# bassamlab/SigmaRL

Measured on AMD Instinct MI355X. Metric: env-steps/sec (agents x envs x steps), CPM scenario, 16 agents (open loop, 32 steps per launch), higher is better.
Workload: dtype f32

## Files before the change

sigmarl_amd/csrc/sigmaenv.hip:

```cpp
#include <hip/hip_runtime.h>

#include <algorithm>
#include <atomic>
#include <cmath>
#include <cstdio>
#include <cstdlib>
#include <cstring>
#include <string>
#include <type_traits>
#include <vector>

#include "sigmaenv_device.h"

using namespace sigmadev;

#ifdef SIGMAENV_PROFILE
#define PROF_TS2(g, tid, k) do { if ((g).dbg_ts2 && (tid) == 0) (g).dbg_ts2[(size_t)blockIdx.x * 16 + (k)] = __builtin_readcyclecounter(); } while (0)
#else
#define PROF_TS2(g, tid, k) do { } while (0)
#endif

#include "../../include/sigmaenv_ref_weights.h"
static_assert(NS >= 1 && NS <= SIGMAENV_MAX_SHORT_TERM, "SIGMAENV_N_SHORT_TERM out of range");
__device__ __constant__ uint32_t W_REF_BITS[NS] = SIGMAENV_W_REF_BITS;
// ... 1032 lines not shown
  for (int k = threadIdx.x; k < t.slots * NS * 2; k += blockDim.x) s.shrt[k] = g.short_term[t.a0 * NS * 2 + k];
  for (int k = threadIdx.x; k < t.slots; k += blockDim.x) s.dref[k] = g.dist_ref[t.a0 + k];
  for (int k = threadIdx.x; k < t.slots * 5; k += blockDim.x) { s.dleft[k] = g.dist_left[t.a0 * 5 + k]; s.dright[k] = g.dist_right[t.a0 * 5 + k]; }
  for (int k = threadIdx.x; k < t.slots * N; k += blockDim.x) s.dist[(k / N) * DIST_STRIDE(N) + (k % N)] = g.dist_agents[t.a0 * N + k];
  for (int k = threadIdx.x; k < t.slots; k += blockDim.x) {
    float psi = g.state[(t.a0 + k) * 8 + 2];
    s.cs[k * 2] = cr_cos(psi);
    s.cs[k * 2 + 1] = cr_sin(psi);
    s.path[k] = g.path[(t.a0 + k) * 4];
    s.cp[k * 3 + 0] = g.closest[(t.a0 + k) * 3 + 0]; s.cp[k * 3 + 1] = g.closest[(t.a0 + k) * 3 + 1]; s.cp[k * 3 + 2] = g.closest[(t.a0 + k) * 3 + 2];
    s.fresh[k] = g.fresh ? g.fresh[t.a0 + k] : 0;
  }
  __syncthreads();
}

__global__ void __launch_bounds__(256) sigmaenv_observe_kernel(sigmaenv_config_t c, DevBufs g, int G) {
  sigma_poison_lds();
  extern __shared__ __attribute__((aligned(16))) char smem_raw[];
  const Tile t(c, G);
  Smem s(smem_raw, G * t.N, t.N, t.K, t.DL);
  load_tile_for_observation(s, g, t);
  observe_tile(c, s, g, t);
}

__global__ void sigmaenv_reset_scatter_kernel(DevBufs g, int N, int n, const int32_t* env_idx, const int32_t* agent_idx, const int32_t* path_ids,
                                              const float* state8, int full_env) {
  sigma_poison_lds();
  int k = blockIdx.x * blockDim.x + threadIdx.x;
  if (k >= n) return;
  int b = env_idx[k], i = agent_idx[k];
  size_t bi = (size_t)b * N + i;
  for (int q = 0; q < 8; ++q) g.state[bi * 8 + q] = state8[(size_t)k * 8 + q];
  for (int q = 0; q < 4; ++q) g.path[bi * 4 + q] = path_ids[(size_t)k * 4 + q];
  if (g.fresh) g.fresh[bi] = 1;
  atomicOr(&g.reset_mask[b], 1ull << i);
  if (full_env) g.reset_full[b] = 1;
}

template <bool WAVE = false, bool VARIANTS = true>
__device__ inline void reset_finish_body(const sigmaenv_config_t& c, const DevBufs& g, const Smem& s, const Tile& t,
                                         const unsigned long long* agent_mask, const int* full, int with_obs, int g_cap = 64, int* lds_tim = nullptr,
                                         const CfgDerived* dvp = nullptr, bool fin = true);
__device__ inline void reset_derive_body(const sigmaenv_config_t& c, const DevMap& m, const DevBufs& g, const Smem& s, const Tile& t,
                                         const unsigned long long* agent_mask, const int* full, int with_obs) {
  const int N = t.N;
  const int tid = threadIdx.x, lane = tid & 63, wave = tid >> 6, n_waves = blockDim.x >> 6;
#define TS2(k) PROF_TS2(g, tid, k)
  for (int sl = tid; sl < t.slots; sl += blockDim.x) {
    int e = sl / N, i = sl - e * N;
    if ((agent_mask[e] >> i) & 1ull) {
      float v[10];
      rect_vertices(c, s.st[sl * 8], s.st[sl * 8 + 1], s.st[sl * 8 + 2], v, &s.cs[sl * 2]);
#pragma unroll
      for (int k = 0; k < 10; ++k) { s.vnew[sl * 10 + k] = v[k]; g.vertices[(t.a0 + sl) * 10 + k] = v[k]; }
    }
  }
  __syncthreads();
  if (m.nch > 0) {
    for (int task = tid; task < t.slots * 3; task += blockDim.x) {
      int sl = task / 3;
      if ((agent_mask[sl / N] >> (sl % N)) & 1ull) scan_mask_task<false>(m, s, task, false, N);
    }
    __syncthreads();
    TS2(3);
    for (int pr = wave; 2 * pr < t.slots; pr += n_waves) {
      int sa = 2 * pr, sb = 2 * pr + 1;
      bool ma = (agent_mask[sa / N] >> (sa % N)) & 1ull;
      bool mb = (sb < t.slots) && ((agent_mask[sb / N] >> (sb % N)) & 1ull);
      if (!(ma || mb)) continue;
      if (m.fast_div) pair_scan<false, true>(m, c, s, sa, (ma ? 1 : 0) | (mb ? 2 : 0), lane, false, N);
      else pair_scan<false, false>(m, c, s, sa, (ma ? 1 : 0) | (mb ? 2 : 0), lane, false, N);
    }
  } else {
    for (int sl = wave; sl < t.slots; sl += n_waves) {
      int e = sl / N, i = sl - e * N;
      if (!((agent_mask[e] >> i) & 1ull)) continue;
      AgentScan r;
      agent_scan_full<false>(m, c, s.path[sl], lane, s.st[sl * 8], s.st[sl * 8 + 1], s.vnew + sl * 10, s.vnew + sl * 10, r);
      if (lane == 0) {
        s.dref[sl] = r.d_ref;
#pragma unroll
        for (int q = 0; q < 5; ++q) { s.dleft[sl * 5 + q] = r.dl[q]; s.dright[sl * 5 + q] = r.dr[q]; }
        s.cp[sl * 3 + 0] = r.cp_ref; s.cp[sl * 3 + 1] = r.cp_l; s.cp[sl * 3 + 2] = r.cp_r;
      }
    }
  }
  __syncthreads();
  TS2(4);
  for (int sl = tid; sl < t.slots; sl += blockDim.x) {
    int e = sl / N, i = sl - e * N;
    if (!((agent_mask[e] >> i) & 1ull)) continue;
    const size_t gi = t.a0 + sl;
    float mbnd = INFINITY;
    g.dist_ref[gi] = s.dref[sl];
#pragma unroll
    for (int q = 0; q < 5; ++q) { g.dist_left[gi * 5 + q] = s.dleft[sl * 5 + q]; g.dist_right[gi * 5 + q] = s.dright[sl * 5 + q]; }
#pragma unroll
    for (int q = 0; q < 5; ++q) mbnd = fminf(mbnd, s.dleft[sl * 5 + q]);
#pragma unroll
    for (int q = 0; q < 5; ++q) mbnd = fminf(mbnd, s.dright[sl * 5 + q]);
    g.dist_bound[gi] = mbnd;
    g.closest[gi * 3 + 0] = s.cp[sl * 3 + 0]; g.closest[gi * 3 + 1] = s.cp[sl * 3 + 1]; g.closest[gi * 3 + 2] = s.cp[sl * 3 + 2];
    int path = s.path[sl];
    float sp[NS * 2];
    short_term_path(m.center + (size_t)path * m.P * 2, m.n_center[path], m.is_loop[path] != 0, s.cp[sl * 3], sp);
#pragma unroll
    for (int k = 0; k < NS * 2; ++k) { g.short_term[gi * NS * 2 + k] = sp[k]; s.shrt[sl * NS * 2 + k] = sp[k]; }
  }
#undef TS2
  reset_finish_body<false>(c, g, s, t, agent_mask, full, with_obs);
}

template <bool WAVE, bool VARIANTS>
__device__ inline void reset_finish_body(const sigmaenv_config_t& c, const DevBufs& g, const Smem& s, const Tile& t,
                                         const unsigned long long* agent_mask, const int* full, int with_obs, int g_cap, int* lds_tim, const CfgDerived* dvp,
                                         bool fin) {
  const int N = t.N;
  const int tid = Grp<WAVE>::tid();
#define TS2(k) PROF_TS2(g, tid, k)
  if (!fin && lds_tim) {
    for (int e = tid; e < t.nenv; e += Grp<WAVE>::size()) {
      if (agent_mask[e] == 0ull) continue;
      const int b = t.env0 + e;
      if (full[e]) {
        const int episodes = lds_tim[e * 4 + 3] + 1;
        lds_tim[e * 4] = 0; lds_tim[e * 4 + 3] = episodes;
        g.timer[b * 4 + 3] = episodes;
      }
      g.reset_mask[b] = 0ull;
      g.reset_full[b] = 0;
    }
    return;
  }
  const float diag = dvp ? dvp->diag : sqrtf(c.world_x_dim * c.world_x_dim + c.world_y_dim * c.world_y_dim);
  for (int p = tid; p < t.slots * N; p += Grp<WAVE>::size()) {
    int si = fdiv(p, g.mN), j = p - si * N;
    int e = fdiv(si, g.mN);
    if (agent_mask[e] == 0ull) continue;
    int sj = e * N + j;
    float d = (si == sj) ? diag : pair_distance(c, s.st, s.vnew, si, sj);
    s.dist[si * DIST_STRIDE(N) + j] = d;
    g.dist_agents[t.a0 * N + p] = d;
    g.col_agents[t.a0 * N + p] = 0;
  }
  for (int sl = tid; sl < t.slots; sl += Grp<WAVE>::size()) {
    int e = sl / N, i = sl - e * N;
    if (agent_mask[e] == 0ull) continue;
    const size_t gi = t.a0 + sl;
    reinterpret_cast<uchar4*>(g.col_flags)[gi] = make_uchar4(0, 0, 0, 0);
    reinterpret_cast<float2*>(g.prev_pos)[gi] = make_float2(s.st[sl * 8], s.st[sl * 8 + 1]);
    if (full[e]) reinterpret_cast<float2*>(g.action)[gi] = make_float2(0.f, 0.f);
    if (i == 0) {
      int b = t.env0 + e;
      if (full[e]) {
        g.timer[b * 4] = 0; g.timer[b * 4 + 3] += 1; g.done[b] = 0;
        if (lds_tim) { lds_tim[e * 4] = 0; lds_tim[e * 4 + 3] += 1; }
      }
      g.reset_mask[b] = 0ull;
      g.reset_full[b] = 0;
    }
  }
  if (with_obs) {
    __threadfence_block();
    Grp<WAVE>::sync();
    TS2(5);
    if (with_obs == 2 && t.nenv == 1 && agent_mask[0]) {
      observe_tile<WAVE, VARIANTS>(c, s, g, t, -1, nullptr, 0, true, lds_tim, dvp);
    } else if (with_obs == 2) {
      int* env_sel = const_cast<int*>(full) + g_cap + 2;
      if (tid == 0) {
        int cnt = 0;
        for (int e = 0; e < t.nenv; ++e) if (agent_mask[e]) env_sel[1 + cnt++] = e;
        env_sel[0] = cnt;
      }
      Grp<WAVE>::sync();
      observe_tile<WAVE, VARIANTS>(c, s, g, t, -1, env_sel + 1, env_sel[0], true, lds_tim, dvp);
    } else {
      load_tile_for_observation(s, g, t);
      observe_tile<WAVE, VARIANTS>(c, s, g, t);
    }
    TS2(6);
  }
#undef TS2
}

__global__ void __launch_bounds__(512) sigmaenv_reset_derive_kernel(sigmaenv_config_t c, DevMap m, DevBufs g, int with_obs, int G) {
  sigma_poison_lds();
  extern __shared__ __attribute__((aligned(16))) char smem_raw[];
  const Tile t(c, G);
  const int N = t.N;
  unsigned long long* s_mask = reinterpret_cast<unsigned long long*>(smem_raw + ((Smem::bytes(G * N, N, t.K, t.DL) + 15) & ~(size_t)15));
  int* s_full = reinterpret_cast<int*>(s_mask + MAX_G);
  int* s_any = s_full + MAX_G;
  if (threadIdx.x == 0) *s_any = 0;
  __syncthreads();
  if (threadIdx.x < t.nenv) {
    unsigned long long mk = g.reset_mask[t.env0 + threadIdx.x];
    s_mask[threadIdx.x] = mk;
    s_full[threadIdx.x] = g.reset_full[t.env0 + threadIdx.x];
    if (mk) *s_any = 1;
  }
  __syncthreads();
  if (!*s_any) return;
  Smem s(smem_raw, G * N, N, t.K, t.DL);
  for (int k = threadIdx.x; k < t.slots * 8; k += blockDim.x) s.st[k] = g.state[t.a0 * 8 + k];
  for (int k = threadIdx.x; k < t.slots * 10; k += blockDim.x) s.vnew[k] = g.vertices[t.a0 * 10 + k];
  for (int k = threadIdx.x; k < t.slots; k += blockDim.x) {
    s.path[k] = g.path[(t.a0 + k) * 4];
    s.fresh[k] = g.fresh ? g.fresh[t.a0 + k] : 0;
    int pt = g.path[(t.a0 + k) * 4 + 3];
    s.cp[k * 3 + 0] = pt; s.cp[k * 3 + 1] = pt; s.cp[k * 3 + 2] = pt;
  }
  __syncthreads();
  reset_derive_body(c, m, g, s, t, s_mask, s_full, with_obs);
}

__global__ void __launch_bounds__(256) sigmaenv_start_table_kernel(sigmaenv_config_t c, DevMap m, float* table) {
  sigma_poison_lds();
  extern __shared__ __attribute__((aligned(16))) char smem_raw[];
  const int S = 64;
  Smem s(smem_raw, S, 1, 0, 1);
  const int tid = threadIdx.x, lane = tid & 63, wave = tid >> 6, n_waves = blockDim.x >> 6;
  __shared__ unsigned long long s_valid;
  __shared__ float s_cosv[64], s_sinv[64];
  const int total = m.n_paths * m.P;
  const int idx = blockIdx.x * S + lane;
  const int path = idx < total ? idx / m.P : 0, pt = idx < total ? idx - (idx / m.P) * m.P : 0;
  const bool valid = idx < total && pt < m.n_center[path];
  if (wave == 0) {
    const unsigned long long vb = __ballot(valid);
    if (lane == 0) s_valid = vb;
    const int sl = lane;
    float x = 0.f, y = 0.f, rot = 0.f;
    if (valid) {
      x = m.center[((size_t)path * m.P + pt) * 2];
      y = m.center[((size_t)path * m.P + pt) * 2 + 1];
      rot = m.yaw[(size_t)path * m.yaw_stride + (pt < m.yaw_stride ? pt : m.yaw_stride - 1)];
    }
    s.st[sl * 8] = x; s.st[sl * 8 + 1] = y; s.st[sl * 8 + 2] = rot;
    float v[10];
    rect_vertices(c, x, y, rot, v, &s.cs[sl * 2]);
#pragma unroll
    for (int k = 0; k < 10; ++k) s.vnew[sl * 10 + k] = v[k];
    s.path[sl] = path;
    s.cp[sl * 3] = pt; s.cp[sl * 3 + 1] = pt; s.cp[sl * 3 + 2] = pt;
    s_cosv[sl] = cr_cos(0.0f + rot);
    s_sinv[sl] = cr_sin(0.0f + rot);
  }
  __syncthreads();
  const unsigned long long vm = s_valid;
  if (m.nch > 0) {
    for (int task = tid; task < S * 3; task += blockDim.x) {
      if ((vm >> (task / 3)) & 1ull) scan_mask_task<false>(m, s, task, false, 1);
    }
    __syncthreads();
    for (int pr = wave; 2 * pr < S; pr += n_waves) {
      const int va = (int)((vm >> (2 * pr)) & 1ull), vb = (int)((vm >> (2 * pr + 1)) & 1ull);
      if (!(va || vb)) continue;
      if (m.fast_div) pair_scan<false, true>(m, c, s, 2 * pr, va | (vb << 1), lane, false, 1);
      else pair_scan<false, false>(m, c, s, 2 * pr, va | (vb << 1), lane, false, 1);
    }
  } else {
    for (int sl = wave; sl < S; sl += n_waves) {
      if (!((vm >> sl) & 1ull)) continue;
      AgentScan r;
      agent_scan_full<false>(m, c, s.path[sl], lane, s.st[sl * 8], s.st[sl * 8 + 1], s.vnew + sl * 10, s.vnew + sl * 10, r);
      if (lane == 0) {
        s.dref[sl] = r.d_ref;
#pragma unroll
        for (int q = 0; q < 5; ++q) { s.dleft[sl * 5 + q] = r.dl[q]; s.dright[sl * 5 + q] = r.dr[q]; }
        s.cp[sl * 3 + 0] = r.cp_ref; s.cp[sl * 3 + 1] = r.cp_l; s.cp[sl * 3 + 2] = r.cp_r;
      }
    }
  }
  __syncthreads();
  if (wave == 0 && idx < total) {
    const int sl = lane;
    float* row = table + (size_t)idx * START_ROW;
    for (int k = 0; k < START_ROW; ++k) row[k] = 0.0f;
    if (valid) {
      row[START_X] = s.st[sl * 8]; row[START_X + 1] = s.st[sl * 8 + 1]; row[START_X + 2] = s.st[sl * 8 + 2];
      row[START_COSV] = s_cosv[sl]; row[START_COSV + 1] = s_sinv[sl];
      for (int k = 0; k < 10; ++k) row[START_VERT + k] = s.vnew[sl * 10 + k];
      row[START_CS] = s.cs[sl * 2]; row[START_CS + 1] = s.cs[sl * 2 + 1];
      row[START_DREF] = s.dref[sl];
      float mbnd = INFINITY;
      for (int q = 0; q < 5; ++q) { row[START_DLEFT + q] = s.dleft[sl * 5 + q]; row[START_DRIGHT + q] = s.dright[sl * 5 + q]; }
      for (int q = 0; q < 5; ++q) mbnd = fminf(mbnd, s.dleft[sl * 5 + q]);
      for (int q = 0; q < 5; ++q) mbnd = fminf(mbnd, s.dright[sl * 5 + q]);
      row[START_DBOUND] = mbnd;
      float sp[NS * 2];
      short_term_path(m.center + (size_t)path * m.P * 2, m.n_center[path], m.is_loop[path] != 0, s.cp[sl * 3], sp);
      for (int k = 0; k < NS * 2; ++k) row[START_SHORT + k] = sp[k];
      for (int k = 0; k < 3; ++k) row[START_CP + k] = __int_as_float(s.cp[sl * 3 + k]);
    }
  }
}

__device__ __forceinline__ void place_from_start_table(const DevMap& m, const DevBufs& g, const Smem& s, const Tile& t, int sl, int path, int pt,
                                                       float speed, int path_first, bool full_env, int scenario_id = 0, bool fin = true) {
  const float4* row4 = reinterpret_cast<const float4*>(m.start_table + ((size_t)path * m.P + pt) * START_ROW);
  float r[START_ROW];
#pragma unroll
  for (int k = 0; k < START_ROW / 4; ++k) { float4 q = row4[k]; r[4 * k] = q.x; r[4 * k + 1] = q.y; r[4 * k + 2] = q.z; r[4 * k + 3] = q.w; }
  const size_t gi = t.a0 + sl;
  const float st[8] = {r[START_X], r[START_X + 1], r[START_X + 2], speed, 0.0f, speed * r[START_COSV], speed * r[START_COSV + 1], 0.0f};
  if (fin) {
    float4* gs = reinterpret_cast<float4*>(g.state + gi * 8);
    gs[0] = make_float4(st[0], st[1], st[2], st[3]);
    gs[1] = make_float4(st[4], st[5], st[6], st[7]);
  }
#pragma unroll
  for (int k = 0; k < 8; ++k) s.st[sl * 8 + k] = st[k];
#pragma unroll
  for (int k = 0; k < 5; ++k) {
    s.vnew[sl * 10 + 2 * k] = r[START_VERT + 2 * k]; s.vnew[sl * 10 + 2 * k + 1] = r[START_VERT + 2 * k + 1];
    if (fin) reinterpret_cast<float2*>(g.vertices + gi * 10)[k] = make_float2(r[START_VERT + 2 * k], r[START_VERT + 2 * k + 1]);
  }
  s.cs[sl * 2] = r[START_CS]; s.cs[sl * 2 + 1] = r[START_CS + 1];
  s.carry[sl * 3] = 0.0f; s.carry[sl * 3 + 1] = r[START_CS]; s.carry[sl * 3 + 2] = r[START_CS + 1] + 0.0f;
  if (fin) {
    s.dref[sl] = r[START_DREF];
    g.dist_ref[gi] = r[START_DREF];
#pragma unroll
    for (int q = 0; q < 5; ++q) {
      s.dleft[sl * 5 + q] = r[START_DLEFT + q]; s.dright[sl * 5 + q] = r[START_DRIGHT + q];
      g.dist_left[gi * 5 + q] = r[START_DLEFT + q]; g.dist_right[gi * 5 + q] = r[START_DRIGHT + q];
    }
    s.dbound[sl] = r[START_DBOUND];
    g.dist_bound[gi] = r[START_DBOUND];
  }
#pragma unroll
  for (int k = 0; k < NS; ++k) {
    s.shrt[sl * NS * 2 + 2 * k] = r[START_SHORT + 2 * k]; s.shrt[sl * NS * 2 + 2 * k + 1] = r[START_SHORT + 2 * k + 1];
    if (fin) reinterpret_cast<float2*>(g.short_term + gi * NS * 2)[k] = make_float2(r[START_SHORT + 2 * k], r[START_SHORT + 2 * k + 1]);
  }
#pragma unroll
  for (int k = 0; k < 3; ++k) { const int cpk = __float_as_int(r[START_CP + k]); s.cp[sl * 3 + k] = cpk; if (fin) g.closest[gi * 3 + k] = cpk; }
  s.path[sl] = path;
  s.fresh[sl] = 1;
  if (fin && g.fresh) g.fresh[gi] = 1;
  g.path[gi * 4 + 0] = path;
  if (full_env) g.path[gi * 4 + 1] = scenario_id;
  g.path[gi * 4 + 2] = path - path_first;
  g.path[gi * 4 + 3] = pt;
}

template <bool WAVE, bool VARIANTS>
__device__ __forceinline__ void auto_reset_tile(const sigmaenv_config_t& c, const DevMap& m, const DevBufs& g, const Smem& s, const Tile& t,
                                       const unsigned long long* s_mask, const int* s_full, uint64_t seed, uint64_t counter, int path_first,
                                       int path_count, int obs_mode, const ResetPrefetch& pre, int g_cap, int* lds_tim, const CfgDerived* dvp, bool fin_arg) {
  const bool fin = fin_arg || !lds_tim;
  const int N = t.N;
  const int tid = Grp<WAVE>::tid(), lane = tid & 63, wave = tid >> 6, n_waves = Grp<WAVE>::size() >> 6;
  const bool mixed = path_count < 0;
  ResetDraw rd{seed, counter, path_first, path_count, c.is_testing_mode, c.env_index_base};
#define TS2(k) PROF_TS2(g, tid, k)
  TS2(1);
  float min_d_sq;
  if (dvp) {
    min_d_sq = dvp->min_d_sq;
  } else {
    const float min_d = sqrtf((float)((double)c.length * (double)c.length + (double)c.width * (double)c.width)) * 1.5f;
    min_d_sq = min_d * min_d;
  }
  const int TR = 64 / N > 0 ? 64 / N : 1;
  for (int e = wave; e < t.nenv; e += n_waves) {
    const int b = t.env0 + e;
    if (!s_full[e]) {
      unsigned long long rq = s_mask[e];
      while (rq) {
        const int i = __ffsll((long long)rq) - 1;
        rq &= rq - 1ull;
        const int sl = e * N + i;
        int p2, q2;
        float x2, y2;
        if (mixed) scenario_list(m, g.path[(t.a0 + sl) * 4 + 1], rd.path_first, rd.path_count);
        reset_candidate(m, rd, b, i, lane, p2, q2, x2, y2, DRAW_AGENT_TRY);
        bool ok = true;
        for (int j = 0; j < N; ++j) {
          if (j == i) continue;
          float dx = x2 - s.st[(e * N + j) * 8], dy = y2 - s.st[(e * N + j) * 8 + 1];
          float d2 = dx * dx + dy * dy;
          if (!(d2 >= min_d_sq)) ok = false;
        }
        unsigned long long f2 = __ballot(ok);
        const int wl = f2 ? (__ffsll((long long)f2) - 1) : (AUTO_RESET_MAX_TRIES - 1);
        if (lane == wl) {
          float u = rng_uniform(rng_u32(seed, counter, (uint32_t)(c.env_index_base + b), (uint32_t)i, DRAW_AGENT_SPEED));
          place_from_start_table(m, g, s, t, sl, p2, q2, u * c.max_speed, rd.path_first, false, 0, fin);
        }
        __builtin_amdgcn_fence(__ATOMIC_RELEASE, "wavefront");
        __builtin_amdgcn_wave_barrier();
        __builtin_amdgcn_fence(__ATOMIC_ACQUIRE, "wavefront");
      }
      continue;
    }
    int sid = 0;
    if (mixed) {
      sid = draw_scenario(m, seed, counter, c.env_index_base + b);
      scenario_list(m, sid, rd.path_first, rd.path_count);
    }
    const int ca = lane / TR, ctr = lane - ca * TR;
    const bool has_c = ca < N;
    int cpath = 0, cpt = 3;
    float cx = 0.f, cy = 0.f;
    if (pre.have && e == wave) { cpath = pre.path; cpt = pre.pt; cx = pre.x; cy = pre.y; }
    else if (has_c) reset_candidate(m, rd, b, ca, ctr, cpath, cpt, cx, cy);
    bool cok = has_c;
    int my_path = 0, my_pt = 3;
    for (int i = 0; i < N; ++i) {
      unsigned long long feas = __ballot(cok && ca == i);
      int path, pt;
      float px, py;
      if (feas) {
        const int wl = __builtin_amdgcn_readfirstlane(__ffsll((long long)feas) - 1);
        path = __builtin_amdgcn_readlane(cpath, wl); pt = __builtin_amdgcn_readlane(cpt, wl);
        px = __int_as_float(__builtin_amdgcn_readlane(__float_as_int(cx), wl)); py = __int_as_float(__builtin_amdgcn_readlane(__float_as_int(cy), wl));
      } else {
        int p2, q2;
        float x2, y2;
        reset_candidate(m, rd, b, i, lane, p2, q2, x2, y2);
        bool ok = lane >= TR;
        wave_sync();
        for (int j = 0; j < i; ++j) {
          float dx = x2 - s.st[(e * N + j) * 8], dy = y2 - s.st[(e * N + j) * 8 + 1];
          float d2 = dx * dx + dy * dy;
          if (!(d2 >= min_d_sq)) ok = false;
        }
        unsigned long long f2 = __ballot(ok);
        const int wl = __builtin_amdgcn_readfirstlane(f2 ? (__ffsll((long long)f2) - 1) : (AUTO_RESET_MAX_TRIES - 1));
        path = __builtin_amdgcn_readlane(p2, wl); pt = __builtin_amdgcn_readlane(q2, wl);
        px = __int_as_float(__builtin_amdgcn_readlane(__float_as_int(x2), wl)); py = __int_as_float(__builtin_amdgcn_readlane(__float_as_int(y2), wl));
      }
      if (lane == i) { my_path = path; my_pt = pt; }
      if (lane == 0) { s.st[(e * N + i) * 8] = px; s.st[(e * N + i) * 8 + 1] = py; }
      float dx = cx - px, dy = cy - py;
      float d2 = dx * dx + dy * dy;
      if (ca > i && !(d2 >= min_d_sq)) cok = false;
    }
    if (lane < N) {
      const int i = lane, sl = e * N + i;
      float u = rng_uniform(rng_u32(seed, counter, (uint32_t)(c.env_index_base + b), (uint32_t)i, DRAW_RESET_SPEED));
      place_from_start_table(m, g, s, t, sl, my_path, my_pt, u * c.max_speed, rd.path_first, true, sid, fin);
    }
  }
  __threadfence_block();
  Grp<WAVE>::sync();
  TS2(2);
  reset_finish_body<WAVE, VARIANTS>(c, g, s, t, s_mask, s_full, obs_mode, g_cap, lds_tim, dvp, fin);
#undef TS2
}

#include "sigmaenv_step_wave.inc"

__global__ void __launch_bounds__(512) sigmaenv_auto_reset_kernel(sigmaenv_config_t c, DevMap m, DevBufs g, uint64_t seed, uint64_t counter,
                                                                  int path_first, int path_count, int G) {
  sigma_poison_lds();
  extern __shared__ __attribute__((aligned(16))) char smem_raw[];
  const Tile t(c, G);
  const int N = t.N;
  const int tid = threadIdx.x;
  unsigned long long* s_mask = reinterpret_cast<unsigned long long*>(smem_raw + ((Smem::bytes(G * N, N, t.K, t.DL) + 15) & ~(size_t)15));
  int* s_full = reinterpret_cast<int*>(s_mask + MAX_G);
  int* s_any = s_full + MAX_G;
#define TS2(k) PROF_TS2(g, tid, k)
#ifdef SIGMAENV_PROFILE
  if (g.dbg_ts2 && tid < 16) g.dbg_ts2[(size_t)blockIdx.x * 16 + tid] = 0ull;
#endif
  TS2(0);
#undef TS2
  if (tid == 0) *s_any = 0;
  __syncthreads();
  if (tid < t.nenv) {
    const int dn = g.done[t.env0 + tid];
    unsigned long long rq = 0ull;
    if (!dn && (c.is_testing_mode || c.has_entry_exit)) {
      for (int i = 0; i < N; ++i) rq |= (unsigned long long)(g.col_flags[((size_t)(t.env0 + tid) * N + i) * 4 + 3] != 0) << i;
    }
    s_mask[tid] = dn ? ((N >= 64) ? ~0ull : ((1ull << N) - 1ull)) : rq;
    s_full[tid] = dn;
    if (dn || rq) *s_any = 1;
  }
  __syncthreads();
  if (!*s_any) return;
  Smem s(smem_raw, G * N, N, t.K, t.DL);
  for (int k = tid; k < t.slots * 8; k += blockDim.x) s.st[k] = g.state[t.a0 * 8 + k];
  for (int k = tid; k < t.slots * 10; k += blockDim.x) s.vnew[k] = g.vertices[t.a0 * 10 + k];
  for (int k = tid; k < t.slots; k += blockDim.x) { s.path[k] = g.path[(t.a0 + k) * 4]; s.fresh[k] = g.fresh ? g.fresh[t.a0 + k] : 0; }
  __syncthreads();
  ResetPrefetch none;
  none.have = false;
  auto_reset_tile(c, m, g, s, t, s_mask, s_full, seed, counter, path_first, path_count, (G == 1 && s_full[0]) ? 2 : 1, none);
}

struct sigmaenv_eval;
struct sigmaenv {
  sigmaenv_config_t cfg;
  int device = 0;
  hipStream_t stream = nullptr;
  int B = 0, N = 0, K = 0, D = 0, P = 0, n_paths = 0;
  DevMap map{};
  DevBufs buf{};
  std::vector<void*> allocs;
  size_t smem_bytes = 0;
  int block = 256;
  int reset_block = 256;
  int G = 1;
  int wave_G = 1, wave_wpb = 1, wave_grid = 1;
  size_t wave_tile_lds = 0;
  int wave_spec = 0;
  sigmaenv_config_t* d_cfg = nullptr;
  DevConfig cfg_derived;
  uint32_t observe_calls = 0;
  size_t rollout_slab_stride = 0;
  float* rollout_obs_rec = nullptr;
  size_t rollout_obs_stride = 0;
  uint32_t* learn_minmax = nullptr;
  float* episode_ws = nullptr;
  int grid = 1;
  void* bufs[SIGMAENV_BUF_COUNT] = {nullptr};
  size_t buf_bytes[SIGMAENV_BUF_COUNT] = {0};
  int32_t *d_env_idx = nullptr, *d_agent_idx = nullptr, *d_path_ids = nullptr;
  float* d_state8 = nullptr;
  size_t staging_cap = 0;
  struct KernelTimer {
    std::vector<std::pair<hipEvent_t, hipEvent_t>> pool;
    std::vector<int> used;
    unsigned long long launch_count = 0;
  };
  KernelTimer timers[SIGMAENV_KERNEL_COUNT];
  bool timing = false;
  int timing_stride = 8;
  sigmaenv_cbf_config_t cbf_cfg{};
  void *cbf_seg4 = nullptr, *cbf_segl = nullptr, *cbf_cxy = nullptr, *cbf_u = nullptr, *cbf_kin = nullptr, *cbf_clf = nullptr, *cbf_safe = nullptr;
  int cbf_seg_stride = 0;
  const float* cbf_centers_inject = nullptr;
  float* lanelet_centers = nullptr;
  unsigned long long* lanelet_neigh = nullptr;
  int n_lanelets = 0, lanelet_pts = 0;
  int DL = 0;
  void* cbf_defer = nullptr;
  void* cbf_cand_big = nullptr;
  int32_t* cbf_groups = nullptr;
  bool cbf_groups_valid = false;
  void* wrap_ws = nullptr;
  size_t wrap_ws_bytes = 0;
  sigmaenv_eval* eval_attached = nullptr;
  std::vector<sigmaenv_eval*> evals;
  std::string err;
};

#define HIPCHK(h, call)                                                                              \
  do {                                                                                               \
    hipError_t e_ = (call);                                                                          \
    if (e_ != hipSuccess) {                                                                          \
      (h)->err = std::string(#call) + ": " + hipGetErrorString(e_);                                  \
      return SIGMAENV_EHIP;                                                                          \
    }                                                                                                \
  } while (0)

static int dev_alloc(sigmaenv* h, void** p, size_t bytes, bool scratch = false) {
  if (bytes == 0) bytes = 16;
  hipError_t e = hipMalloc(p, bytes);
  if (e != hipSuccess) { h->err = std::string("hipMalloc: ") + hipGetErrorString(e); return SIGMAENV_ENOMEM; }
  h->allocs.push_back(*p);
#ifdef SIGMAENV_POISON
  e = hipMemsetAsync(*p, scratch ? 0xFF : 0, bytes, h->stream);
#else
  (void)scratch;
  e = hipMemsetAsync(*p, 0, bytes, h->stream);
#endif
  if (e != hipSuccess) { h->err = std::string("hipMemsetAsync: ") + hipGetErrorString(e); return SIGMAENV_EHIP; }
  return SIGMAENV_OK;
}

static void dev_free(sigmaenv* h, void* p) {
  if (!p) return;
  for (size_t k = 0; k < h->allocs.size(); ++k)
    if (h->allocs[k] == p) { h->allocs.erase(h->allocs.begin() + (long)k); break; }
  (void)hipFree(p);
}

extern "C" int sigmaenv_n_short_term(void) { return NS; }
#ifndef SIGMAENV_BUILD_ID
#define SIGMAENV_BUILD_ID "unknown"
#endif
extern "C" const char* sigmaenv_build_id(void) { return SIGMAENV_BUILD_ID; }
extern "C" int sigmaenv_obs_dim(int32_t n_nearing) { return 1 + 2 * NS + 3 + n_nearing * 11; }
extern "C" int sigmaenv_obs_dim_ex(int32_t n_nearing, int32_t f) {
  const int s = (f & SIGMAENV_OBS_STEERING) ? 1 : 0, r = (f & SIGMAENV_OBS_REF_OTHERS) ? 1 : 0;
  const int own = 1 + s + 2 * NS + ((f & SIGMAENV_OBS_NO_DIST_CENTER) ? 0 : 1) + ((f & SIGMAENV_OBS_BOUNDARY_POINTS) ? 20 : 2) + ((f & SIGMAENV_OBS_BIRD_VIEW) ? 4 : 0);
  const int other = ((f & SIGMAENV_OBS_NO_VERTICES) ? 5 : 8) + 2 + s + ((f & SIGMAENV_OBS_NO_DIST_AGENTS) ? 0 : 1) + r * 2 * NS;
  return own + n_nearing * other + ((f & SIGMAENV_OBS_OPPONENT_PAD) ? 2 * n_nearing : 0);
}

extern "C" int sigmaenv_obs_dim_full(int32_t n_agents, int32_t n_nearing, int32_t f) {
  if (!(f & SIGMAENV_OBS_FULL)) return sigmaenv_obs_dim_ex(n_nearing, f);
  if (!(f & SIGMAENV_OBS_BIRD_VIEW) || n_nearing < 1 || n_agents < 1) return SIGMAENV_EINVAL;
  const int N = n_agents, K = n_nearing;
  int wid[9], nf = 0;
  if (!(f & SIGMAENV_OBS_NO_VERTICES)) wid[nf++] = 8; else { wid[nf++] = 2; wid[nf++] = 1; wid[nf++] = 1; wid[nf++] = 1; }
  wid[nf++] = 2;
  if (f & SIGMAENV_OBS_STEERING) wid[nf++] = 1;
  if (!(f & SIGMAENV_OBS_NO_DIST_AGENTS)) wid[nf++] = N;
  if (f & SIGMAENV_OBS_REF_OTHERS) wid[nf++] = 2 * NS;
  if (N % K != 0) return SIGMAENV_EINVAL;
  int others = 0;
  for (int q = 0; q < nf; ++q) {
    if ((N * wid[q]) % K != 0) return SIGMAENV_EINVAL;
    others += N * wid[q];
  }
  return sigmaenv_obs_dim_ex(0, f & ~SIGMAENV_OBS_OPPONENT_PAD) + others + ((f & SIGMAENV_OBS_OPPONENT_PAD) ? 2 * K : 0);
}

extern "C" const char* sigmaenv_last_error(const sigmaenv_t* h) { return h ? h->err.c_str() : "null handle"; }

static void eval_orphan(sigmaenv* h);

extern "C" void sigmaenv_destroy(sigmaenv_t* h) {
  if (!h) return;
  (void)hipSetDevice(h->device);
  (void)hipStreamSynchronize(h->stream);
  eval_orphan(h);
  for (void* p : h->allocs) (void)hipFree(p);
  for (auto& tm : h->timers)
    for (auto& ev : tm.pool) { (void)hipEventDestroy(ev.first); (void)hipEventDestroy(ev.second); }
  delete h;
}

static int pick_envs_per_group(int N, int B, int n_cu) {
  int G = 64 / N;
  if (G < 1) G = 1;
  if (G > MAX_G) G = MAX_G;
  while (G > 1 && (B + G - 1) / G < 4 * n_cu) G >>= 1;
  return G;
}

#ifdef SIGMAENV_POISON
__global__ void sigma_poison_probe_kernel(unsigned* out) {
  extern __shared__ char probe_smem[];
  if (threadIdx.x == 0) { probe_smem[0] = 1; out[0] = sigma_lds_alloc_units() + (probe_smem[0] ? 0u : 1u); }
}
static int poison_probe(hipStream_t stream) {
  static bool done = false;
  if (done) return SIGMAENV_OK;
  unsigned* d = nullptr;
  unsigned units[2] = {0u, 0u};
  if (hipMalloc((void**)&d, 8) != hipSuccess) return SIGMAENV_ENOMEM;
  hipLaunchKernelGGL(sigma_poison_probe_kernel, dim3(1), dim3(64), 32768, stream, d);
  hipLaunchKernelGGL(sigma_poison_probe_kernel, dim3(1), dim3(64), 16384, stream, d + 1);
  if (hipMemcpyAsync(units, d, 8, hipMemcpyDeviceToHost, stream) != hipSuccess || hipStreamSynchronize(stream) != hipSuccess) { (void)hipFree(d); return SIGMAENV_EHIP; }
  (void)hipFree(d);
  unsigned granule = 0u;
  for (unsigned g : {64u, 128u, 256u, 512u})
    if (units[0] * g >= 32768u && units[0] * g < 32768u + 2048u && units[1] * g >= 16384u && units[1] * g < 16384u + 2048u) granule = g;
  if (granule == 0u) {
    fprintf(stderr, "sigmaenv (poison build): unexpected LDS_ALLOC.LDS_SIZE readings %u / %u for 32768 / 16384 bytes\n", units[0], units[1]);
    return SIGMAENV_EHIP;
  }
  if (hipMemcpyToSymbol(HIP_SYMBOL(sigmadev::sigma_lds_granule), &granule, sizeof(unsigned)) != hipSuccess) return SIGMAENV_EHIP;
  fprintf(stderr, "sigmaenv (poison build): LDS and scratch buffers are poisoned (LDS_SIZE unit = %u bytes)\n", granule);
  done = true;
  return SIGMAENV_OK;
}
#endif

extern "C" int sigmaenv_create(const sigmaenv_config_t* cfg, const sigmaenv_map_t* map, int device_id, void* hip_stream, sigmaenv_t** out) {
  if (!cfg || !map || !out) return SIGMAENV_EINVAL;
  *out = nullptr;
  if (cfg->abi_version != SIGMAENV_ABI_VERSION) return SIGMAENV_EINVAL;
  for (int k = 0; k < 3; ++k) if (cfg->reserved[k] != 0) return SIGMAENV_EINVAL;
  if (cfg->n_points_short_term != 0 && cfg->n_points_short_term != NS) {
    fprintf(stderr, "sigmaenv_create: n_points_short_term = %d, but this library is built for %d (make -C sigmarl_amd/csrc NS=%d)\n", cfg->n_points_short_term, NS, cfg->n_points_short_term);
    return SIGMAENV_EINVAL;
  }
  if (cfg->env_index_base < 0 || !(cfg->obs_noise_level >= 0.0f)) return SIGMAENV_EINVAL;
  if (cfg->n_envs < 1 || cfg->n_agents < 1 || cfg->n_agents > SIGMAENV_MAX_AGENTS) return SIGMAENV_EINVAL;
  if (cfg->n_nearing < 0 || cfg->n_nearing > SIGMAENV_MAX_NEARING || cfg->n_nearing > cfg->n_agents - 1) return SIGMAENV_EINVAL;
  if (cfg->distance_type != SIGMAENV_DIST_C2C && cfg->distance_type != SIGMAENV_DIST_MTV) return SIGMAENV_EINVAL;
  if (map->n_paths < 1 || map->stride_points < 2) return SIGMAENV_EINVAL;
  int n_dev = 0;
  if (hipGetDeviceCount(&n_dev) != hipSuccess || n_dev < 1 || device_id < 0 || device_id >= n_dev) return SIGMAENV_ENODEV;
  if (hipSetDevice(device_id) != hipSuccess) return SIGMAENV_ENODEV;
#ifdef SIGMAENV_POISON
  { const int rcp = poison_probe(reinterpret_cast<hipStream_t>(hip_stream)); if (rcp != SIGMAENV_OK) return rcp; }
#endif
  sigmaenv* h = new sigmaenv();
  h->cfg = *cfg;
  h->device = device_id;
  h->stream = reinterpret_cast<hipStream_t>(hip_stream);
  const int B = h->B = cfg->n_envs, N = h->N = cfg->n_agents, K = h->K = cfg->n_nearing;
  h->D = sigmaenv_obs_dim_full(N, K, cfg->obs_flags);
  if (h->D < 0) { delete h; return SIGMAENV_EINVAL; }
  h->DL = h->D;
  if (cfg->obs_flags != 0) {
    const ObsLayout L(cfg->obs_flags, N, K);
    if (L.D != h->D) { delete h; return SIGMAENV_EINVAL; }
    h->DL = L.DL;
  }
  const int np = h->n_paths = map->n_paths, S = map->stride_points;
  for (int p = 0; p < np; ++p) {
    if (map->n_center[p] < 2 || map->n_left[p] < 2 || map->n_right[p] < 2 || map->n_center[p] > S || map->n_left[p] > S || map->n_right[p] > S) {
      delete h;
      return SIGMAENV_EINVAL;
    }
  }
  int maxc = 0;
  for (int p = 0; p < np; ++p) maxc = map->n_center[p] > maxc ? map->n_center[p] : maxc;
  int P = maxc + NS * 2 + 2;
  for (int p = 0; p < np; ++p) {
    if (map->n_left[p] > P) P = map->n_left[p];
    if (map->n_right[p] > P) P = map->n_right[p];
  }
  h->P = P;
  std::vector<float> hc((size_t)np * P * 2), hl((size_t)np * P * 2), hr((size_t)np * P * 2);
  for (int p = 0; p < np; ++p) {
    const int n = map->n_center[p], nl = map->n_left[p], nr = map->n_right[p];
    const float* c = map->center + (size_t)p * S * 2;
    float* dc = hc.data() + (size_t)p * P * 2;
    memcpy(dc, c, (size_t)n * 8);
    const float dirx = c[2 * (n - 1)] - c[2 * (n - 2)], diry = c[2 * (n - 1) + 1] - c[2 * (n - 2) + 1];
    const int ne = NS * 2;
    for (int k = 1; k <= ne; ++k) {
      volatile float kx = (float)k * dirx, ky = (float)k * diry;
      dc[2 * (n + k - 1)] = c[2 * (n - 1)] + kx;
      dc[2 * (n + k - 1) + 1] = c[2 * (n - 1) + 1] + ky;
    }
    for (int k = n + ne; k < P; ++k) { dc[2 * k] = dc[2 * (n + ne - 1)]; dc[2 * k + 1] = dc[2 * (n + ne - 1) + 1]; }
    const float* l = map->left + (size_t)p * S * 2;
    float* dl = hl.data() + (size_t)p * P * 2;
    memcpy(dl, l, (size_t)nl * 8);
    for (int k = nl; k < P; ++k) { dl[2 * k] = l[2 * (nl - 1)]; dl[2 * k + 1] = l[2 * (nl - 1) + 1]; }
    const float* r = map->right + (size_t)p * S * 2;
    float* dr = hr.data() + (size_t)p * P * 2;
    memcpy(dr, r, (size_t)nr * 8);
    for (int k = nr; k < P; ++k) { dr[2 * k] = r[2 * (nr - 1)]; dr[2 * k + 1] = r[2 * (nr - 1) + 1]; }
  }
  int rc;
#define ALLOC(ptr, bytes)                                         \
  if ((rc = dev_alloc(h, (void**)&(ptr), (bytes))) != SIGMAENV_OK) { \
    std::string e = h->err;                                       \
    sigmaenv_destroy(h);                                          \
    fprintf(stderr, "sigmaenv_create: %s\n", e.c_str());        \
    return rc;                                                    \
  }
  float *d_c, *d_l, *d_r, *d_y;
  int32_t *d_nc, *d_nl, *d_nr;
// ... 630 lines not shown
```

sigmarl_amd/csrc/sigmaenv_device.h:

```cpp
#pragma once

#include <hip/hip_runtime.h>
#include <stdint.h>

#include "../../include/sigmaenv.h"
#include "../../include/sigma_trig_f32.h"
#include "sigmaenv_dist.h"

#define NS SIGMAENV_N_SHORT_TERM
#define PI32 3.14159274101257324f
#define TWO_PI32 (2.0f * PI32)

namespace sigmadev {

#ifdef SIGMAENV_POISON
__device__ unsigned sigma_lds_granule = 0u;
__device__ __forceinline__ unsigned sigma_lds_alloc_units() { return (unsigned)__builtin_amdgcn_s_getreg(6 | (12 << 6) | ((9 - 1) << 11)); }
__device__ __forceinline__ void sigma_poison_lds() {
  const unsigned words = sigma_lds_alloc_units() * sigma_lds_granule / 4u;
  auto* lds = (__attribute__((address_space(3))) unsigned*)0;
  const unsigned tid = threadIdx.x + blockDim.x * (threadIdx.y + blockDim.y * threadIdx.z), nt = blockDim.x * blockDim.y * blockDim.z;
  for (unsigned k = tid; k < words; k += nt) lds[k] = 0xFFFFFFFFu;
  __syncthreads();
}
#else
__device__ __forceinline__ void sigma_poison_lds() {}
#endif

struct DevMap {
  const float* center;
  const float* left;
  const float* right;
  const float* yaw;
  const int32_t* n_center;
  const int32_t* n_left;
  const int32_t* n_right;
  const uint8_t* is_loop;
  int32_t P, n_paths, yaw_stride;
  const float4* chunk_box;
  const float4* group_box;
  const ulonglong4* chunk_neigh;
  float neigh_radius, neigh_radius_far;
  int32_t nch;
  const float* start_table;
  int32_t fast_div;
  float rect_radius;
  int32_t poly_stride;
  int32_t n_lists;
  float cdf0, cdf1, cdf2;
  float neigh_radius_tight;
  unsigned long long list_first16, list_count16;
};
#define SIGMAENV_CHUNK 4
struct CfgDerived {
  float l_wb;
  float k_beta;
  float lh, wh;
  float diag;
  float rew_denom;
  float r_pos, r_v, r_dl;
  float r_wx, r_wy;
  float min_d_sq;
};
struct DevConfig {
  sigmaenv_config_t c;
  CfgDerived d;
};
inline CfgDerived derive_config(const sigmaenv_config_t& c) {
  CfgDerived d;
  d.l_wb = (float)((double)c.l_f + (double)c.l_r);
  d.k_beta = (float)((double)c.l_r / ((double)c.l_f + (double)c.l_r));
  d.lh = (float)((double)c.length / 2.0);
  d.wh = (float)((double)c.width / 2.0);
  const float xx = c.world_x_dim * c.world_x_dim, yy = c.world_y_dim * c.world_y_dim;
  d.diag = sqrtf(xx + yy);
  d.rew_denom = (float)((double)c.max_speed * (double)c.dt);
  const float n_pos = (float)((double)c.length * 10.0), n_v = c.max_speed, n_dl = (float)((double)c.lane_width * 3.0);
  d.r_pos = 1.0f / n_pos; d.r_v = 1.0f / n_v; d.r_dl = 1.0f / n_dl;
  d.r_wx = 1.0f / c.world_x_dim; d.r_wy = 1.0f / c.world_y_dim;
  const float min_d = sqrtf((float)((double)c.length * (double)c.length + (double)c.width * (double)c.width)) * 1.5f;
  d.min_d_sq = min_d * min_d;
  return d;
}

#define START_X 0
#define START_COSV 3
#define START_VERT 5
#define START_CS 15
#define START_DREF 17
#define START_DLEFT 18
#define START_DRIGHT 23
#define START_DBOUND 28
#define START_SHORT 29
#define START_CP (START_SHORT + 2 * NS)
#define START_ROW ((START_CP + 3 + 3) & ~3)

struct DevBufs {
  float *state, *prev_pos, *vertices, *short_term, *dist_ref, *dist_left, *dist_right, *dist_bound, *dist_agents;
  float *reward, *reward_info, *obs, *action, *cbf_nominal;
  int32_t *path, *closest, *nearing, *timer;
  uint8_t *col_agents, *col_flags, *done;
  unsigned long long* reset_mask;
  uint8_t* reset_full;
  uint8_t* fresh;
  float* slab;
  const float* lanelet_centers;
  const unsigned long long* lanelet_neigh;
  int32_t n_lanelets, lanelet_pts;
  const float* bnd_left;
  const int32_t* bnd_n_center;
  const uint8_t* bnd_is_loop;
  int32_t bnd_poly_stride, bnd_P;
  uint32_t mVT1;
  uint32_t obs_salt;
  uint32_t mN, mT1, mT2, mTP, mW, mSG;
  int dbg_skip;
  unsigned long long* dbg_ts2;
  unsigned long long* dbg_ts;
};

struct __attribute__((packed, aligned(8))) Seg4 { float ax, ay, bx, by; };
__device__ __forceinline__ Seg4 load_segment(const float2* p, int k) { return *reinterpret_cast<const Seg4*>(p + k); }

__host__ __device__ constexpr uint32_t magic_u32(unsigned d) { return d <= 1u ? 0u : (uint32_t)(((1ull << 32) + d - 1ull) / d); }
__device__ __forceinline__ int fdiv(int x, uint32_t m) { return m ? (int)__umulhi((uint32_t)x, m) : x; }

struct __attribute__((packed, aligned(4))) F4u { float x, y, z, w; };

__device__ __forceinline__ float cr_sin(float x) { return sigma_sinf(x); }
__device__ __forceinline__ float cr_cos(float x) { return sigma_cosf(x); }
__device__ __forceinline__ float cr_tan(float x) { return sigma_tanf(x); }
__device__ __forceinline__ float cr_atan(float x) { return sigma_atanf(x); }
__device__ __forceinline__ void cr_sincos(float x, float& s, float& c) { sigma_sincosf(x, &s, &c); }
__device__ __forceinline__ float norm2(float x, float y) { return sqrtf(fmaf(y, y, x * x)); }
__device__ __forceinline__ float clampf(float x, float lo, float hi) { return fminf(fmaxf(x, lo), hi); }
__device__ __forceinline__ float fmin_nc(float a, float b) {
  float r;
  asm("v_min_f32 %0, %1, %2" : "=v"(r) : "v"(a), "v"(b));
  return r;
}
__device__ __forceinline__ float remainder_pos(float a, float b) {
  if (a >= 0.0f && a < b) return a;
  float m = fmodf(a, b);
  if (m != 0.0f && m < 0.0f) m += b;
  return m;
}
__device__ __forceinline__ float angle_eliminate_two_pi(float a) {
  float r = remainder_pos(a, TWO_PI32);
  if (r > PI32) r -= TWO_PI32;
  return r;
}
__device__ __forceinline__ float decreasing_lin(float x, float x0, float x1) {
  x = clampf(x, x0, x1);
  float denom = x1 - x0;
  return 1.0f - (x - x0) / denom;
}

__device__ inline void bicycle_step(const sigmaenv_config_t& c, float s[8], float u0, float u1, float uc[2]) {
  float a0 = clampf(u0, -c.max_speed, c.max_speed);
  float a1 = clampf(u1, -c.max_steering, c.max_steering);
  uc[0] = a0;
  uc[1] = a1;
  float x = s[0], y = s[1], psi = s[2], v = s[3], delta = s[4];
  float u_acc = (a0 - v) / c.dt;
  float u_sr = (a1 - delta) / c.dt;
  u_acc = clampf(u_acc, c.min_acc, c.max_acc);
  u_sr = clampf(u_sr, c.min_steering_rate, c.max_steering_rate);
  float l_wb = (float)((double)c.l_f + (double)c.l_r);
  float k_beta = (float)((double)c.l_r / ((double)c.l_f + (double)c.l_r));
  float tan_d = cr_tan(delta);
  float beta = cr_atan(k_beta * tan_d);
  float s0, c0;
  cr_sincos(psi + beta, s0, c0);
  float dx0 = v * c0;
  float dx1 = v * s0;
  float dx2 = (v / l_wb) * tan_d * cr_cos(beta);
  float dt = c.dt;
  x = x + dt * dx0;
  y = y + dt * dx1;
  psi = psi + dt * dx2;
  v = v + dt * u_acc;
  delta = delta + dt * u_sr;
  delta = remainder_pos(delta + PI32, TWO_PI32) - PI32;
  float beta1 = cr_atan(k_beta * cr_tan(delta));
  float course = psi + beta1;
  s[0] = x; s[1] = y; s[2] = psi; s[3] = v; s[4] = delta;
  float s1, c1;
  cr_sincos(course, s1, c1);
  s[5] = v * c1;
  s[6] = v * s1;
  s[7] = beta1;
}

__device__ inline void rect_vertices(const sigmaenv_config_t& c, float px, float py, float psi, float* v , float* cs_out = nullptr) {
  float lh = (float)((double)c.length / 2.0), wh = (float)((double)c.width / 2.0);
  float cs, sn;
  cr_sincos(psi, sn, cs);
  if (cs_out) { cs_out[0] = cs; cs_out[1] = sn; }
  float nsn = -sn;
  const float bx[5] = {lh, lh, -lh, -lh, lh};
  const float by[5] = {wh, -wh, -wh, wh, wh};
#pragma unroll
  for (int k = 0; k < 5; ++k) {
    v[2 * k] = (cs * bx[k] + nsn * by[k]) + px;
    v[2 * k + 1] = (sn * bx[k] + cs * by[k]) + py;
  }
}

__device__ __forceinline__ float point_segment(float px, float py, float sx, float sy, float lx, float ly, float len2) {
  float vx = px - sx, vy = py - sy;
  float proj = (vx * lx + vy * ly) / len2;
  float t = clampf(proj, 0.0f, 1.0f);
  float cx = sx + lx * t, cy = sy + ly * t;
  return norm2(cx - px, cy - py);
}

__device__ __forceinline__ float point_segment_sq(float px, float py, float sx, float sy, float lx, float ly, float len2) {
  float vx = px - sx, vy = py - sy;
  float proj = (vx * lx + vy * ly) / len2;
  float t = clampf(proj, 0.0f, 1.0f);
  float cx = sx + lx * t, cy = sy + ly * t;
  float ex = cx - px, ey = cy - py;
  return fmaf(ey, ey, ex * ex);
}

__device__ __forceinline__ float shared_rcp(float b) {
  float y0 = __builtin_amdgcn_rcpf(b);
  float e = fmaf(-b, y0, 1.0f);
  return fmaf(e, y0, y0);
}
__device__ __forceinline__ float div_shared(float a, float b, float y) {
  float q = a * y;
  float r = fmaf(-b, q, a);
  q = fmaf(r, y, q);
  r = fmaf(-b, q, a);
  return fmaf(r, y, q);
}
template <bool FAST>
__device__ __forceinline__ float point_segment_t(float px, float py, float sx, float sy, float lx, float ly, float len2, float rcp) {
  float vx = px - sx, vy = py - sy;
  float num = vx * lx + vy * ly;
  float proj = FAST ? div_shared(num, len2, rcp) : num / len2;
  float t = clampf(proj, 0.0f, 1.0f);
  float cx = sx + lx * t, cy = sy + ly * t;
  return norm2(cx - px, cy - py);
}
template <bool FAST>
__device__ __forceinline__ float point_segment_sq_t(float px, float py, float sx, float sy, float lx, float ly, float len2, float rcp) {
  float vx = px - sx, vy = py - sy;
  float num = vx * lx + vy * ly;
  float proj = FAST ? div_shared(num, len2, rcp) : num / len2;
  float t = clampf(proj, 0.0f, 1.0f);
  float cx = sx + lx * t, cy = sy + ly * t;
  float ex = cx - px, ey = cy - py;
  return fmaf(ey, ey, ex * ex);
}

struct Edge {
  float xa, ya, xb, yb, dx, dy, S;
};
__device__ __forceinline__ Edge make_edge(float xa, float ya, float xb, float yb) {
  Edge e;
  e.xa = xa; e.ya = ya; e.xb = xb; e.yb = yb;
  e.dx = xb - xa;
  e.dy = yb - ya;
  e.S = e.dx * ya - e.dy * xa;
  return e;
}
__device__ __forceinline__ bool edge_hits_segment(const Edge& e, float x2a, float y2a, float x2b, float y2b, float dx2, float dy2, float S2) {
  float ma = e.dx * y2a - e.dy * x2a, mb = e.dx * y2b - e.dy * x2b;
  bool C1 = ((ma - e.S) * (mb - e.S)) < 0.0f;
  float wa = e.ya * dx2 - e.xa * dy2, wb = e.yb * dx2 - e.xb * dy2;
  bool C2 = ((wa - S2) * (wb - S2)) < 0.0f;
  return C1 && C2;
}
__device__ inline bool interx_rect_seg(const float* v, float x2a, float y2a, float x2b, float y2b) {
  float dx2 = x2b - x2a, dy2 = y2b - y2a;
  float S2 = dx2 * y2a - dy2 * x2a;
  bool hit = false;
#pragma unroll
  for (int i = 0; i < 4; ++i) {
    Edge e = make_edge(v[2 * i], v[2 * i + 1], v[2 * i + 2], v[2 * i + 3]);
    hit |= edge_hits_segment(e, x2a, y2a, x2b, y2b, dx2, dy2, S2);
  }
  return hit;
}

__device__ inline void rect_axes(const float* v, float ax[2][2]) {
#pragma unroll
  for (int k = 0; k < 2; ++k) {
    float ex = v[2 * (k + 1)] - v[2 * k], ey = v[2 * (k + 1) + 1] - v[2 * k + 1];
    float nrm = norm2(ex, ey);
    ax[k][0] = ex / nrm;
    ax[k][1] = ey / nrm;
  }
}
__device__ inline void mtv_half(const float* va, const float* vb, const float axb[2][2], float& pos_min, float& omin_out, bool& any_inside) {
  float maxbb[2], minbb[2], maxab[2], minab[2], pab[4][2];
#pragma unroll
  for (int k = 0; k < 2; ++k) {
    maxbb[k] = -INFINITY; minbb[k] = INFINITY; maxab[k] = -INFINITY; minab[k] = INFINITY;
#pragma unroll
    for (int v = 0; v < 4; ++v) {
      float pb = vb[2 * v] * axb[k][0] + vb[2 * v + 1] * axb[k][1];
      float pa = va[2 * v] * axb[k][0] + va[2 * v + 1] * axb[k][1];
      pab[v][k] = pa;
      maxbb[k] = fmaxf(maxbb[k], pb); minbb[k] = fminf(minbb[k], pb);
      maxab[k] = fmaxf(maxab[k], pa); minab[k] = fminf(minab[k], pa);
    }
  }
  float ov0 = fminf(maxbb[0], maxab[0]) - fmaxf(minbb[0], minab[0]);
  float ov1 = fminf(maxbb[1], maxab[1]) - fmaxf(minbb[1], minab[1]);
  float omin = fminf(ov0, ov1);
  omin_out = omin;
  bool inside_any = false;
  float pm = INFINITY;
#pragma unroll
  for (int v = 0; v < 4; ++v) {
    float g[2];
    bool inside = true;
#pragma unroll
    for (int k = 0; k < 2; ++k) {
      float p = pab[v][k];
      g[k] = (p - minbb[k]) * (p <= minbb[k] ? 1.0f : 0.0f) + (maxbb[k] - p) * (p >= maxbb[k] ? 1.0f : 0.0f);
      inside = inside && (p > minbb[k]) && (p < maxbb[k]);
    }
    pm = fminf(pm, norm2(g[0], g[1]));
    float neg = -omin * (inside ? 1.0f : 0.0f);
    if (fabsf(neg) > 0.0f) inside_any = true;
  }
  pos_min = pm;
  any_inside = inside_any;
}
#define MTV_REC 8
__device__ inline void rect_mtv_record(const float* v, float* rec) {
  float ax[2][2];
  rect_axes(v, ax);
#pragma unroll
  for (int k = 0; k < 2; ++k) {
    float mx = -INFINITY, mn = INFINITY;
#pragma unroll
    for (int q = 0; q < 4; ++q) {
      const float pb = v[2 * q] * ax[k][0] + v[2 * q + 1] * ax[k][1];
      mx = fmaxf(mx, pb); mn = fminf(mn, pb);
    }
    rec[2 * k] = ax[k][0]; rec[2 * k + 1] = ax[k][1];
    rec[4 + k] = mn; rec[6 + k] = mx;
  }
}
__device__ inline void mtv_half_staged(const float* va, const float* recb, float& pos_min, float& omin_out, bool& any_inside) {
  float maxbb[2], minbb[2], maxab[2], minab[2], pab[4][2];
#pragma unroll
  for (int k = 0; k < 2; ++k) {
    maxbb[k] = recb[6 + k]; minbb[k] = recb[4 + k]; maxab[k] = -INFINITY; minab[k] = INFINITY;
#pragma unroll
    for (int v = 0; v < 4; ++v) {
      float pa = va[2 * v] * recb[2 * k] + va[2 * v + 1] * recb[2 * k + 1];
      pab[v][k] = pa;
      maxab[k] = fmaxf(maxab[k], pa); minab[k] = fminf(minab[k], pa);
    }
  }
  float ov0 = fminf(maxbb[0], maxab[0]) - fmaxf(minbb[0], minab[0]);
  float ov1 = fminf(maxbb[1], maxab[1]) - fmaxf(minbb[1], minab[1]);
  float omin = fminf(ov0, ov1);
  omin_out = omin;
  bool inside_any = false;
  float pm = INFINITY;
#pragma unroll
  for (int v = 0; v < 4; ++v) {
    float g[2];
    bool inside = true;
#pragma unroll
    for (int k = 0; k < 2; ++k) {
      float p = pab[v][k];
      g[k] = (p - minbb[k]) * (p <= minbb[k] ? 1.0f : 0.0f) + (maxbb[k] - p) * (p >= maxbb[k] ? 1.0f : 0.0f);
      inside = inside && (p > minbb[k]) && (p < maxbb[k]);
    }
    pm = fminf(pm, norm2(g[0], g[1]));
    float neg = -omin * (inside ? 1.0f : 0.0f);
    if (fabsf(neg) > 0.0f) inside_any = true;
  }
  pos_min = pm;
  any_inside = inside_any;
}
__device__ inline float mtv_pair_staged(const float* vi, const float* vj, const float* reci, const float* recj) {
  float pij, pji, omin_j, omin_i;
  bool neg_ij, neg_ji;
  mtv_half_staged(vi, recj, pij, omin_j, neg_ij);
  mtv_half_staged(vj, reci, pji, omin_i, neg_ji);
  float d = fminf(pij, pji);
  if (neg_ij || neg_ji) d = -fminf(omin_j, omin_i);
  return d;
}
__device__ inline float mtv_pair(const float* vi, const float* vj) {
  float axi[2][2], axj[2][2], pij, pji, omin_j, omin_i;
  bool neg_ij, neg_ji;
  rect_axes(vi, axi);
  rect_axes(vj, axj);
// ... 93 lines not shown
```

Baseline: 3.194 billion.

## Rework reset placement to use lane masks and register shuffles instead of LDS

```diff
diff --git a/sigmarl_amd/csrc/sigmaenv.hip b/sigmarl_amd/csrc/sigmaenv.hip
--- a/sigmarl_amd/csrc/sigmaenv.hip
+++ b/sigmarl_amd/csrc/sigmaenv.hip
@@ -1358,7 +1358,11 @@
   const float4* row4 = reinterpret_cast<const float4*>(m.start_table + ((size_t)path * m.P + pt) * START_ROW);
   float r[START_ROW];
 #pragma unroll
-  for (int k = 0; k < START_ROW / 4; ++k) { float4 q = row4[k]; r[4 * k] = q.x; r[4 * k + 1] = q.y; r[4 * k + 2] = q.z; r[4 * k + 3] = q.w; }
+  for (int k = 0; k < START_HOT / 4; ++k) { float4 q = row4[k]; r[4 * k] = q.x; r[4 * k + 1] = q.y; r[4 * k + 2] = q.z; r[4 * k + 3] = q.w; }
+  if (fin) {
+#pragma unroll
+    for (int k = START_HOT / 4; k < START_ROW / 4; ++k) { float4 q = row4[k]; r[4 * k] = q.x; r[4 * k + 1] = q.y; r[4 * k + 2] = q.z; r[4 * k + 3] = q.w; }
+  }
   const size_t gi = t.a0 + sl;
   const float st[8] = {r[START_X], r[START_X + 1], r[START_X + 2], speed, 0.0f, speed * r[START_COSV], speed * r[START_COSV + 1], 0.0f};
   if (fin) {
@@ -1463,43 +1467,52 @@
     float cx = 0.f, cy = 0.f;
     if (pre.have && e == wave) { cpath = pre.path; cpt = pre.pt; cx = pre.x; cy = pre.y; }
     else if (has_c) reset_candidate(m, rd, b, ca, ctr, cpath, cpt, cx, cy);
-    bool cok = has_c;
+    TS2(7);
+    unsigned long long cokm = __ballot(has_c);
+    const unsigned long long tr_mask = ~0ull >> (64 - TR);
+    int my_wl = -1;
     int my_path = 0, my_pt = 3;
+    float my_x = 0.f, my_y = 0.f;
     for (int i = 0; i < N; ++i) {
-      unsigned long long feas = __ballot(cok && ca == i);
-      int path, pt;
+      const unsigned long long feas = (cokm >> (i * TR)) & tr_mask;
       float px, py;
       if (feas) {
-        const int wl = __builtin_amdgcn_readfirstlane(__ffsll((long long)feas) - 1);
-        path = __builtin_amdgcn_readlane(cpath, wl); pt = __builtin_amdgcn_readlane(cpt, wl);
+        const int wl = i * TR + __ffsll((long long)feas) - 1;
         px = __int_as_float(__builtin_amdgcn_readlane(__float_as_int(cx), wl)); py = __int_as_float(__builtin_amdgcn_readlane(__float_as_int(cy), wl));
+        if (lane == i) my_wl = wl;
       } else {
         int p2, q2;
         float x2, y2;
         reset_candidate(m, rd, b, i, lane, p2, q2, x2, y2);
-        bool ok = lane >= TR;
-        wave_sync();
-        for (int j = 0; j < i; ++j) {
-          float dx = x2 - s.st[(e * N + j) * 8], dy = y2 - s.st[(e * N + j) * 8 + 1];
+        unsigned long long f2 = TR < 64 ? ~0ull << TR : 0ull;
+        const float wx = __shfl(cx, my_wl), wy = __shfl(cy, my_wl);
+        const float ax = my_wl >= 0 ? wx : my_x, ay = my_wl >= 0 ? wy : my_y;
+        for (int j = 0; j < i && f2; ++j) {
+          const float axj = __int_as_float(__builtin_amdgcn_readlane(__float_as_int(ax), j)), ayj = __int_as_float(__builtin_amdgcn_readlane(__float_as_int(ay), j));
+          float dx = x2 - axj, dy = y2 - ayj;
           float d2 = dx * dx + dy * dy;
-          if (!(d2 >= min_d_sq)) ok = false;
+          f2 &= __ballot(d2 >= min_d_sq);
         }
-        unsigned long long f2 = __ballot(ok);
         const int wl = __builtin_amdgcn_readfirstlane(f2 ? (__ffsll((long long)f2) - 1) : (AUTO_RESET_MAX_TRIES - 1));
-        path = __builtin_amdgcn_readlane(p2, wl); pt = __builtin_amdgcn_readlane(q2, wl);
+        const int path = __builtin_amdgcn_readlane(p2, wl), pt = __builtin_amdgcn_readlane(q2, wl);
         px = __int_as_float(__builtin_amdgcn_readlane(__float_as_int(x2), wl)); py = __int_as_float(__builtin_amdgcn_readlane(__float_as_int(y2), wl));
+        if (lane == i) { my_path = path; my_pt = pt; my_x = px; my_y = py; }
       }
-      if (lane == i) { my_path = path; my_pt = pt; }
-      if (lane == 0) { s.st[(e * N + i) * 8] = px; s.st[(e * N + i) * 8 + 1] = py; }
       float dx = cx - px, dy = cy - py;
       float d2 = dx * dx + dy * dy;
-      if (ca > i && !(d2 >= min_d_sq)) cok = false;
+      cokm &= __ballot(d2 >= min_d_sq) | (~0ull >> (64 - (i + 1) * TR));
+    }
+    TS2(8);
+    {
+      const int wpath = __shfl(cpath, my_wl), wpt = __shfl(cpt, my_wl);
+      if (my_wl >= 0) { my_path = wpath; my_pt = wpt; }
     }
     if (lane < N) {
       const int i = lane, sl = e * N + i;
       float u = rng_uniform(rng_u32(seed, counter, (uint32_t)(c.env_index_base + b), (uint32_t)i, DRAW_RESET_SPEED));
       place_from_start_table(m, g, s, t, sl, my_path, my_pt, u * c.max_speed, rd.path_first, true, sid, fin);
     }
+    TS2(9);
   }
   __threadfence_block();
   Grp<WAVE>::sync();
diff --git a/sigmarl_amd/csrc/sigmaenv_device.h b/sigmarl_amd/csrc/sigmaenv_device.h
--- a/sigmarl_amd/csrc/sigmaenv_device.h
+++ b/sigmarl_amd/csrc/sigmaenv_device.h
@@ -87,13 +87,14 @@
 #define START_COSV 3
 #define START_VERT 5
 #define START_CS 15
-#define START_DREF 17
-#define START_DLEFT 18
-#define START_DRIGHT 23
-#define START_DBOUND 28
-#define START_SHORT 29
+#define START_SHORT 17
 #define START_CP (START_SHORT + 2 * NS)
-#define START_ROW ((START_CP + 3 + 3) & ~3)
+#define START_HOT ((START_CP + 3 + 3) & ~3)
+#define START_DREF START_HOT
+#define START_DLEFT (START_DREF + 1)
+#define START_DRIGHT (START_DLEFT + 5)
+#define START_DBOUND (START_DRIGHT + 5)
+#define START_ROW ((START_DBOUND + 1 + 3) & ~3)
 
 struct DevBufs {
   float *state, *prev_pos, *vertices, *short_term, *dist_ref, *dist_left, *dist_right, *dist_bound, *dist_agents;
```

After: 3.248 billion, median of 6. 1.7% higher.
